# Vigilans/GomokuAI

Measured on AMD Instinct MI355X. Metric: board-evals/s, higher is better.
Workload: dtype int32

## Files before the change

gomokuai_amd/csrc/eval_kernel.hip:

```cpp
#include <algorithm>
#include <cstdlib>
#include <vector>

#include "capi_common.h"

namespace {

constexpr int kBoardsPerBlock = 16;
constexpr int kGroupBoards = 16;
constexpr int kThreads = 64 * kBoardsPerBlock;
constexpr int kCells = 225;
constexpr int kQueueCap = 448;
constexpr int kMaxBlocksPerCu = 1;

constexpr int kScoreWords = 4 * kCells;
constexpr int kCntWords = 3 * kCells + 1;
constexpr int kZeroWords = kScoreWords + kCntWords;
constexpr int kLineWords = 96;
constexpr int kColBase = 20, kDiagBase = 36, kAntiBase = 65;
#ifndef GMK_K1_TOTALS_COPIES
#define GMK_K1_TOTALS_COPIES 8
#endif
constexpr int kTotalsCopies = GMK_K1_TOTALS_COPIES;
constexpr int kMiscWords = 48;
constexpr int kBoardWords = kZeroWords + kLineWords + kQueueCap + kMiscWords;
static_assert(kZeroWords % 4 == 0 && kBoardWords % 4 == 0, "16-byte alignment of the per-board blocks");
constexpr int kStaticTableWords = 128 + kLineWords + 512 + 1560 + 4;

__constant__ uint32_t c_lane_jobs[64 * 2];
__constant__ uint32_t c_line_init[kLineWords];
__constant__ uint4 c_lane_consts[64];
constexpr int kScanSteps = 19;

__device__ __forceinline__ int dir_stride(int dir) { return (0x0E100F01u >> (8 * dir)) & 0xFFu; }

__device__ __forceinline__ uint64_t line_symbols(uint32_t line_word, int len) {
    return 2ull | (static_cast<uint64_t>(line_word) << 2) | (0xAull << (2 * len + 2));
}

__device__ __forceinline__ const __attribute__((address_space(3))) uint32_t* lds_word(uint32_t byte_address) {
    return reinterpret_cast<const __attribute__((address_space(3))) uint32_t*>(static_cast<uintptr_t>(byte_address));
}

__device__ __forceinline__ __attribute__((address_space(3))) uint32_t* lds_word_rw(uint32_t byte_address) {
    return reinterpret_cast<__attribute__((address_space(3))) uint32_t*>(static_cast<uintptr_t>(byte_address));
}

__device__ __forceinline__ uint32_t dfa_address(uint32_t table_word, uint32_t four) {
    uint32_t addr;
    asm("v_bfi_b32 %0, %1, %2, %3" : "=v"(addr) : "s"(0x3FF3u), "v"(table_word), "v"(four));
// ... 57 lines not shown

__device__ __forceinline__ void add_counter_cells(uint32_t w0, int back, int q, int stride, uint32_t* opp) {
    const int n_dep = (w0 >> 8) & 7, endcell = q + back * stride;
#pragma unroll
    for (int d = 0; d < 4; ++d) {
        const uint32_t f = (w0 >> (11 + 4 * d)) & 15u;
        if (d < n_dep && static_cast<int>(f & 7u) != back) atomicAdd(&opp[4 * (endcell - static_cast<int>(f & 7u) * stride)], 600u);
    }
}

[[maybe_unused]] constexpr int kDensTiles = 7;
__host__ __device__ constexpr int dens_kt_lo(int m) { return (((32 * m) / 15 - 3) < 0 ? 0 : (32 * m) / 15 - 3) / 2; }
__host__ __device__ constexpr int dens_kt_hi(int m) { return (((32 * m + 31) / 15 + 3) > 14 ? 14 : (32 * m + 31) / 15 + 3) / 2; }
constexpr int kWtabDy = 13, kWtabEntryWords = 4, kWtabKindWords = kWtabDy * 15 * kWtabEntryWords, kWtabWords = 2 * kWtabKindWords;
__host__ __device__ constexpr int block_weight(int dy, int dx) {
    constexpr int w[4][7] = {{1, 3, 4, 0, 4, 3, 1}, {0, 3, 5, 4, 5, 3, 0}, {0, 4, 3, 3, 3, 4, 0}, {2, 0, 0, 1, 0, 0, 2}};
    return w[dy < 0 ? -dy : dy][dx + 3];
}

typedef int v4i __attribute__((ext_vector_type(4)));
typedef int v16i __attribute__((ext_vector_type(16)));

template <bool kFull, int KIND, int M>
__device__ __forceinline__ void density_tile_pass(const uint32_t (&own_rows)[8], int n_live, int lane,
                                                  const v4i* __restrict__ s_wtab, const uint4* __restrict__ s_occ, int32_t* __restrict__ group_out,
                                                  unsigned long long& board_base , const uint2* __restrict__ s_lut, int plane_stride) {
    constexpr int lo = dens_kt_lo(M), hi = dens_kt_hi(M), nk = hi - lo + 1;
    const int n = lane & 31, h = lane >> 5;
    const uint4 occ_lo = s_occ[4 * M + 2 * h], occ_hi = s_occ[4 * M + 2 * h + 1];
    const uint32_t occ[8] = {occ_lo.x, occ_lo.y, occ_lo.z, occ_lo.w, occ_hi.x, occ_hi.y, occ_hi.z, occ_hi.w};
    const int cell = 32 * M + n, yo = (cell * 0x8889) >> 19, xo = cell - 15 * yo;
    const v4i* w = s_wtab + KIND * (kWtabKindWords / kWtabEntryWords) + (2 * lo + h - yo + 6) * 15 + xo;
    v16i acc = {0, 0, 0, 0, 0, 0, 0, 0, 0, 0, 0, 0, 0, 0, 0, 0};
#pragma unroll
    for (int k = 0; k < nk; ++k) {
        const uint32_t r = (own_rows[lo + k] >> (16 * h)) & 0x7FFFu;
        const uint2 b0 = s_lut[r & 255u], b1 = s_lut[r >> 8];
        const v4i stones = {static_cast<int>(b0.x), static_cast<int>(b0.y), static_cast<int>(b1.x), static_cast<int>(b1.y)};
        acc = __builtin_amdgcn_mfma_i32_32x32x32_i8(stones, w[30 * k], acc, 0, 0, 0);
    }
    const uint32_t at = static_cast<uint32_t>(KIND * plane_stride + 32 * M + n + h * (2 * 4 * plane_stride));
    if (kFull) {
        const uint32_t at_white = 4u * at, at_black = 4u * (at + 2u * static_cast<uint32_t>(plane_stride));
#pragma unroll
        for (int i = 0; i < 16; i += 2) {
            const int neg = __builtin_amdgcn_sbfe(static_cast<int>(occ[i / 2]), n, 1);
            store_saddr(at_black, acc[i] ^ neg, board_base);
            store_saddr(at_white, acc[i + 1] ^ neg, board_base);
            board_base += static_cast<long long>(i == 14 ? -13 : i % 4 ? 3 : 1) * (4 * 4 * plane_stride);
            asm volatile("" : "+s"(board_base));
        }
    } else {
        int32_t* out = group_out + at;
#pragma unroll
        for (int i = 0; i < 16; i += 2) {
            const int b = 4 * (i / 4) + (i % 4) / 2;
            const int neg = __builtin_amdgcn_sbfe(static_cast<int>(occ[i / 2]), n, 1);
            asm volatile("" : "+s"(n_live));
            if (b + 2 * h < n_live && plane_stride > 0) {
                out[b * 4 * plane_stride + 1 * 2 * plane_stride] = acc[i] ^ neg;
                out[b * 4 * plane_stride + 0 * 2 * plane_stride] = acc[i + 1] ^ neg;
            }
        }
    }
}

template <bool kFull>
__device__ __forceinline__ void density_planes_out(const uint16_t* __restrict__ planes, int n_boards, int first_board, int lane,
                                                   const v4i* __restrict__ s_wtab, uint32_t* __restrict__ s_occ, int32_t* __restrict__ out_density,
                                                   const uint2* __restrict__ s_lut, int plane_stride) {
    const int n = lane & 31, plane = n & 1, board = first_board + (n >> 1);
    uint32_t own[8], other[8];
    {
        const uint4* p = reinterpret_cast<const uint4*>(planes + static_cast<size_t>(kFull || board < n_boards ? board : first_board) * 32);
        const uint4 a0 = p[plane * 2], a1 = p[plane * 2 + 1], b0 = p[2 - plane * 2], b1 = p[3 - plane * 2];
        own[0] = a0.x; own[1] = a0.y; own[2] = a0.z; own[3] = a0.w; own[4] = a1.x; own[5] = a1.y; own[6] = a1.z; own[7] = a1.w;
        other[0] = b0.x; other[1] = b0.y; other[2] = b0.z; other[3] = b0.w; other[4] = b1.x; other[5] = b1.y; other[6] = b1.z; other[7] = b1.w;
    }
    if ((lane & 33) == 0) {
        const int bg = lane >> 1;
        uint32_t* slot = s_occ + 8 * ((bg >> 1) & 1) + 2 * (bg >> 2) + (bg & 1);
#pragma unroll
        for (int m = 0; m < kDensTiles; ++m) {
            const int y0 = (32 * m) / 15, y1 = (32 * m + 31) / 15;
            uint32_t occ = 0;
#pragma unroll
            for (int y = y0; y <= y1; ++y) {
                const uint32_t both = own[y / 2] | other[y / 2];
                const uint32_t r = ((y & 1) ? both >> 16 : both) & 0x7FFFu;
                const int at = 15 * y - 32 * m;
                occ |= at >= 0 ? r << at : r >> -at;
            }
            slot[16 * m] = occ;
        }
    }
    if ((lane >> 5) == 0 && (kFull || (board < n_boards && plane_stride > 0))) {
        uint32_t c224 = 0, w224 = 0;
#pragma unroll
        for (int dy = -3; dy <= 0; ++dy) {
            const int y = 14 + dy;
            const uint32_t r = (y & 1) ? own[y >> 1] >> 16 : own[y >> 1] & 0xFFFFu;
#pragma unroll
            for (int dx = -3; dx <= 0; ++dx) {
                if (block_weight(dy, dx) == 0) continue;
                const uint32_t bit = (r >> (14 + dx)) & 1u;
                c224 += bit;
                w224 += bit * static_cast<uint32_t>(block_weight(dy, dx));
            }
        }
        const uint32_t neg = 0u - (((own[7] | other[7]) >> 14) & 1u);
        int32_t* out = out_density + static_cast<size_t>(board) * 4 * plane_stride + (1 - plane) * 2 * plane_stride;
        out[224] = static_cast<int32_t>(c224 ^ neg);
        out[plane_stride + 224] = static_cast<int32_t>(w224 ^ neg);
    }
    const int n_live = __builtin_amdgcn_readfirstlane(n_boards - first_board);
    int32_t* group_out = out_density + static_cast<size_t>(first_board) * 4 * plane_stride;
    const uint4* occ_words = reinterpret_cast<const uint4*>(s_occ);
    const unsigned long long group_bits = reinterpret_cast<unsigned long long>(group_out);
    unsigned long long board_base = static_cast<unsigned long long>(static_cast<uint32_t>(__builtin_amdgcn_readfirstlane(static_cast<int>(group_bits >> 32)))) << 32
                                    | static_cast<uint32_t>(__builtin_amdgcn_readfirstlane(static_cast<int>(group_bits)));
    asm volatile("" : "+s"(board_base));
#define GMK_PASS(K, M) density_tile_pass<kFull, K, M>(own, n_live, lane, s_wtab, occ_words, group_out, board_base, s_lut, plane_stride); __builtin_amdgcn_sched_barrier(0);
    GMK_PASS(0, 0) GMK_PASS(1, 0) GMK_PASS(0, 1) GMK_PASS(1, 1) GMK_PASS(0, 2) GMK_PASS(1, 2) GMK_PASS(0, 3) GMK_PASS(1, 3)
    GMK_PASS(0, 4) GMK_PASS(1, 4) GMK_PASS(0, 5) GMK_PASS(1, 5) GMK_PASS(0, 6) GMK_PASS(1, 6)
#undef GMK_PASS
}

__global__ __launch_bounds__(kThreads)
void eval_positions_kernel(const uint16_t* __restrict__ planes, int n_boards, int n_groups,
                           int32_t* __restrict__ out_scores, int32_t* __restrict__ out_density,
                           uint32_t* __restrict__ out_totals, int32_t* __restrict__ out_status,
                           const uint32_t* __restrict__ g_trans, const uint32_t* __restrict__ g_records,
                           int trans_words, int record_words, const uint32_t* __restrict__ g_wtab,
                           int phase_mask_arg, unsigned long long* __restrict__ prof) {
#ifdef GMK_PROFILE
    const int phase_mask = phase_mask_arg;
    unsigned long long t_acc[12] = {0, 0, 0, 0, 0, 0, 0, 0, 0, 0, 0, 0}, t_prev = __builtin_amdgcn_s_memtime();
#define GMK_STAMP(k) do { if (prof) { const unsigned long long t_now_ = __builtin_amdgcn_s_memtime(); t_acc[k] += t_now_ - t_prev; t_prev = t_now_; } } while (0)
#else
    constexpr int phase_mask = 0x7F;
    (void)phase_mask_arg; (void)prof;
#define GMK_STAMP(k) do { } while (0)
#endif
    extern __shared__ __attribute__((aligned(16))) uint32_t lds[];
    const uint4* s_rec = reinterpret_cast<const uint4*>(lds + trans_words);
    uint32_t* s_jobs = lds + trans_words + record_words;

    for (int i = threadIdx.x; i < trans_words; i += kThreads) lds[i] = g_trans[i];
    for (int i = threadIdx.x; i < record_words; i += kThreads) lds[trans_words + i] = g_records[i];
    if (threadIdx.x < 128) s_jobs[threadIdx.x] = c_lane_jobs[threadIdx.x];
    uint32_t* s_pads = s_jobs + 128;
    if (threadIdx.x < kLineWords) s_pads[threadIdx.x] = ~c_line_init[threadIdx.x] & 0xAAAAAAAAu;
    uint2* s_lut = reinterpret_cast<uint2*>(s_jobs + 128 + kLineWords);
    if (threadIdx.x < 256) s_lut[threadIdx.x] = make_uint2(((threadIdx.x & 15u) * 0x204081u) & 0x01010101u, ((threadIdx.x >> 4) * 0x204081u) & 0x01010101u);
    uint32_t* s_wtab_words = s_jobs + 128 + kLineWords + 512;
    for (int i = threadIdx.x; i < kWtabWords; i += kThreads) s_wtab_words[i] = g_wtab[i];
    const v4i* s_wtab = reinterpret_cast<const v4i*>(s_wtab_words);
    uint32_t* s_handout = s_wtab_words + kWtabWords;
    if (threadIdx.x < 4) s_handout[threadIdx.x] = threadIdx.x == 0 ? 2u * kBoardsPerBlock : 0u;

    const int wave = __builtin_amdgcn_readfirstlane(threadIdx.x >> 6), lane0 = threadIdx.x & 63;
    uint32_t* s_scores = lds + trans_words + record_words + kStaticTableWords + wave * kBoardWords;
    uint32_t* s_cnt = s_scores + kScoreWords;
    uint32_t* s_lines = s_scores + kZeroWords;
    uint32_t* s_queue = s_lines + kLineWords;
    uint32_t* s_misc = s_queue + kQueueCap;
#ifndef GMK_K1_TOTALS_HOT
    uint32_t* const my_totals = s_queue + kQueueCap - 8 * kTotalsCopies + (lane0 & (kTotalsCopies - 1)) * 8;
#else
    uint32_t* const my_totals = s_misc + 4;
#endif

    GMK_STAMP(0);

    const bool planes_out = out_density != nullptr && (phase_mask & 64) && !(phase_mask & 1024);
    int lane = lane0;
    const uint32_t job_a = c_lane_jobs[lane * 2], job_b = c_lane_jobs[lane * 2 + 1];
    const uint32_t line_init_lo = c_line_init[lane], line_init_hi = c_line_init[min(64 + lane, kLineWords - 1)];
    const uint4 lane_consts = c_lane_consts[lane];
    const uint32_t cell_row4 = lane_consts.x, cell_col = lane_consts.y, norm_a = lane_consts.z, norm_b = lane_consts.w;
    uint32_t* s_rows = s_misc + 16;
    const uint16_t* row_ptr = planes + (lane & 15);
    uint32_t next_black = 0, next_white = 0, cur_black = 0, cur_white = 0;
    auto fetch_row = [&](int b) {
        const uint16_t* p = row_ptr + static_cast<size_t>(min(b, n_boards - 1)) * 32;
        next_black = p[0];
        next_white = p[16];
    };
    auto take_row = [&](int b) -> uint32_t { return lane < 16 && b < n_boards ? cur_black | (cur_white << 16) : 0u; };

    const int wg_g0 = static_cast<int>(static_cast<long long>(n_groups) * blockIdx.x / gridDim.x);
    const int wg_groups = static_cast<int>(static_cast<long long>(n_groups) * (blockIdx.x + 1) / gridDim.x) - wg_g0;
    const int wg_first = wg_g0 * kGroupBoards, wg_boards = min(wg_groups * kGroupBoards, n_boards - wg_first);
    auto hand_out = [&](int which) -> int {
        uint32_t v = 0;
        if (lane0 == 0) v = atomicAdd(&s_handout[which], 1u);
        return __builtin_amdgcn_readfirstlane(static_cast<int>(v));
    };
    int idx = wave, boards_done = 0;
    if (idx < wg_boards) fetch_row(wg_first + idx);
    asm volatile("" : "+v"(next_black), "+v"(next_white));
#pragma unroll 1
    for (;;) {
        const bool live = idx < wg_boards;
        const int board = wg_first + idx;
        cur_black = next_black; cur_white = next_white;
        int idx_next = idx;
        if (live) { idx_next = boards_done == 0 ? kBoardsPerBlock + wave : hand_out(0); fetch_row(wg_first + min(idx_next, wg_boards - 1)); }
        GMK_STAMP(11);

        if (live) {
            {
                uint4* z = reinterpret_cast<uint4*>(s_cnt) + lane;
    #pragma unroll
                for (int i = 0; i < kCntWords / 4; i += 64)
                    if (i + 64 <= kCntWords / 4 || lane < kCntWords / 4 - i) z[i] = make_uint4(0u, 0u, 0u, 0u);
            }
            s_lines[lane] = line_init_lo;
            if (lane < kLineWords - 64) s_lines[64 + lane] = line_init_hi;
            if (lane < kMiscWords) s_misc[lane] = 0;
#ifndef GMK_K1_TOTALS_HOT
            if (lane < 8 * kTotalsCopies) s_queue[kQueueCap - 8 * kTotalsCopies + lane] = 0;
#endif
            const uint32_t my_row = take_row(board);
            wave_phase_fence();
            {
                uint32_t cnt = static_cast<uint32_t>(__popc(my_row & 0x7FFFu)) | (static_cast<uint32_t>(__popc(my_row >> 16)) << 16);
                cnt += static_cast<uint32_t>(__builtin_amdgcn_update_dpp(0, static_cast<int>(cnt), 0x118, 0xF, 0xF, false));
                cnt += static_cast<uint32_t>(__builtin_amdgcn_update_dpp(0, static_cast<int>(cnt), 0x114, 0xF, 0xF, false));
                cnt += static_cast<uint32_t>(__builtin_amdgcn_update_dpp(0, static_cast<int>(cnt), 0x112, 0xF, 0xF, false));
                cnt += static_cast<uint32_t>(__builtin_amdgcn_update_dpp(0, static_cast<int>(cnt), 0x111, 0xF, 0xF, false));
// ... 230 lines not shown
                        for (int i = 0; i < 8; ++i)
                            if (start + i <= k) tw = *lds_word(dfa_address(tw, __builtin_amdgcn_ubfe(cur, 2 * i, 4)));
                        if ((gmk::dev_trans_kinds(tw) >> tslot) & 1u) {
                            const uint4 rec = s_rec[gmk::dev_trans_record(tw)];
                            const int want = 5 - tslot;
                            hit_back = counter_match(rec.x, k, want);
                            hit_w0 = rec.x;
                            if (hit_back < 0) { hit_back = counter_match(rec.z, k, want); hit_w0 = rec.z; }
                        }
                    }
                    const unsigned long long hits = __ballot(hit_back >= 0);
                    const uint32_t mine = static_cast<uint32_t>(hits >> (7 * grp)) & 0x7Fu;
                    if (hit_back >= 0 && (mine & ((1u << kk) - 1u)) == 0u) add_counter_cells(hit_w0, hit_back, q, stride, s_scores + (c ? 2 : 1));
                }
            }
            wave_phase_fence();
            GMK_STAMP(6);

        }

        asm volatile("" : "+v"(next_black), "+v"(next_white));
        GMK_STAMP(7);

        if (planes_out && (!live || (boards_done & 15) == wave)) {
            for (;;) {
                const int burst = hand_out(1);
                if (burst >= wg_groups) break;
                int lane_p = lane0, first_p = (wg_g0 + burst) * kGroupBoards;
                asm volatile("" : "+v"(lane_p), "+s"(first_p));
                const int plane_stride = (phase_mask & 512) ? 0 : (phase_mask & 256) ? 256 : kCells;
                if (first_p + kGroupBoards <= n_boards && plane_stride > 0) density_planes_out<true>(planes, n_boards, first_p, lane_p, s_wtab, s_queue, out_density, s_lut, plane_stride);
                else density_planes_out<false>(planes, n_boards, first_p, lane_p, s_wtab, s_queue, out_density, s_lut, plane_stride);
                GMK_STAMP(8);
                if (live) break;
            }
        }
        if (!live) break;
        if (live && (phase_mask & 32)) {
            int lane_b = lane;
            asm volatile("" : "+v"(lane_b));
            if (out_scores) {
                int32_t* dst = out_scores + static_cast<size_t>(board) * kScoreWords + lane_b;
                const int4* src = reinterpret_cast<const int4*>(s_scores);
                const int4 v0 = src[lane_b], v1 = src[lane_b + 64], v2 = src[lane_b + 128], v3 = src[min(lane_b + 192, kCells - 1)];
#ifdef GMK_K1_PLAIN_SCORES
#define GMK_STORE(p, v) (*(p) = (v))
#else
#define GMK_STORE(p, v) __builtin_nontemporal_store(v, p)
#endif
                const bool tail = lane_b + 192 < kCells;
                GMK_STORE(dst, v0.x); GMK_STORE(dst + 64, v1.x); GMK_STORE(dst + 128, v2.x); if (tail) GMK_STORE(dst + 192, v3.x);
                GMK_STORE(dst + kCells, v0.y); GMK_STORE(dst + kCells + 64, v1.y); GMK_STORE(dst + kCells + 128, v2.y); if (tail) GMK_STORE(dst + kCells + 192, v3.y);
                GMK_STORE(dst + 2 * kCells, v0.z); GMK_STORE(dst + 2 * kCells + 64, v1.z); GMK_STORE(dst + 2 * kCells + 128, v2.z); if (tail) GMK_STORE(dst + 2 * kCells + 192, v3.z);
                GMK_STORE(dst + 3 * kCells, v0.w); GMK_STORE(dst + 3 * kCells + 64, v1.w); GMK_STORE(dst + 3 * kCells + 128, v2.w); if (tail) GMK_STORE(dst + 3 * kCells + 192, v3.w);
#undef GMK_STORE
            }
            if (out_totals && lane_b < 11) out_totals[static_cast<size_t>(board) * 11 + lane_b] = s_misc[4 + lane_b];
            if (out_status && lane_b == 0) {
                const uint32_t wbits = s_misc[1], stones = s_misc[0];
// ... 73 lines not shown
            for (int xo = 0; xo < 15; ++xo)
                for (int j = 0; j < 15; ++j) {
                    if (std::abs(j - xo) > 3) continue;
                    const int w = block_weight(dy, j - xo);
                    t[((static_cast<size_t>(kind) * kWtabDy + dy + 6) * 15 + xo) * 16 + j] = static_cast<int8_t>(kind == 0 ? (w != 0) : w);
                }
    for (int cell = 0; cell < 224; ++cell)
        for (int kt = dens_kt_lo(cell / 32); kt <= dens_kt_hi(cell / 32); ++kt)
            for (int h = 0; h < 2; ++h) {
                const int dy = 2 * kt + h - cell / 15;
                if (dy < -6 || dy > 6) { gmk::set_error("density weight table: dy %d of cell %d out of range", dy, cell); return GMK_ERR_STATE; }
            }
    for (int cell = 0; cell < 224; ++cell)
        for (int dy = -3; dy <= 3; ++dy) {
            const int y = cell / 15 + dy, m = cell / 32;
            if (y < 0 || y > 14) continue;
            if (y / 2 < dens_kt_lo(m) || y / 2 > dens_kt_hi(m)) { gmk::set_error("density weight table: row %d of cell %d is not covered", y, cell); return GMK_ERR_STATE; }
        }
    GMK_HIP_CHECK(hipMalloc(d_out, t.size()));
    GMK_HIP_CHECK(hipMemcpy(*d_out, t.data(), t.size(), hipMemcpyHostToDevice));
    return GMK_OK;
}

struct Launch { int grid, n_groups; size_t lds; };

Launch plan_launch(int n, const gmk::DeviceState& st) {
    Launch l;
    l.n_groups = (n + kGroupBoards - 1) / kGroupBoards;
    l.grid = std::max(1, std::min(l.n_groups, st.cu_count * kMaxBlocksPerCu));
    l.lds = static_cast<size_t>(kBoardsPerBlock * kBoardWords + st.n_states * 4 + st.n_records * 4 + kStaticTableWords) * 4;
    return l;
}

bool g_jobs_uploaded = false;
uint32_t* g_wtab = nullptr;
}

extern "C" int gmk_eval_batch(const uint16_t* d_planes, int n, int32_t* d_scores, int32_t* d_density,
                              uint32_t* d_totals, int32_t* d_status, void* stream) {
    gmk::DeviceState& st = gmk::device_state();
    if (!st.ready) { gmk::set_error("gmk_init has not succeeded (no CPU fallback)"); return GMK_ERR_STATE; }
    if (n < 0 || (n > 0 && !d_planes)) { gmk::set_error("gmk_eval_batch: bad arguments"); return GMK_ERR_ARG; }
    if (n == 0) return GMK_OK;
    if (!g_jobs_uploaded) {
        int rc = upload_lane_jobs();
        if (rc != GMK_OK) return rc;
        rc = upload_density_weights(&g_wtab);
        if (rc != GMK_OK) return rc;
        GMK_HIP_CHECK(hipFuncSetAttribute(reinterpret_cast<const void*>(eval_positions_kernel), hipFuncAttributeMaxDynamicSharedMemorySize, 160 * 1024));
        g_jobs_uploaded = true;
    }
    const Launch l = plan_launch(n, st);
    if (l.lds > 160u * 1024u) { gmk::set_error("gmk_eval_batch: tables do not fit in LDS (%zu bytes)", l.lds); return GMK_ERR_CAPACITY; }
    static const int phase_mask = gmk::profile_env("GMK_EVAL_PHASE_MASK") ? std::atoi(gmk::profile_env("GMK_EVAL_PHASE_MASK")) : 0x7F;
    unsigned long long* d_prof = nullptr;
    static const bool stamps = gmk::profile_env("GMK_EVAL_PROFILE") != nullptr;
    if (stamps) {
        GMK_HIP_CHECK(hipMalloc(&d_prof, 16 * sizeof(unsigned long long)));
        GMK_HIP_CHECK(hipMemset(d_prof, 0, 16 * sizeof(unsigned long long)));
    }
    hipLaunchKernelGGL(eval_positions_kernel, dim3(l.grid), dim3(kThreads), l.lds, static_cast<hipStream_t>(stream),
                       d_planes, n, l.n_groups, d_scores, d_density, d_totals, d_status,
                       st.d_trans, st.d_records, st.n_states * 4, st.n_records * 4, g_wtab, phase_mask, d_prof);
    GMK_HIP_CHECK(hipGetLastError());
    if (stamps) {
        unsigned long long h[16];
        GMK_HIP_CHECK(hipDeviceSynchronize());
        GMK_HIP_CHECK(hipMemcpy(h, d_prof, sizeof h, hipMemcpyDeviceToHost));
        (void)hipFree(d_prof);
        const char* names[12] = {"staging", "phase0", "scan", "deposits", "phase3", "phase3b", "rescans", "wait-planes", "phaseD", "phase5", "-", "loop-head"};
        const double boards = static_cast<double>(n), waves = static_cast<double>(h[15] ? h[15] : 1);
        double total = 0;
        for (int k = 0; k < 12; ++k) total += static_cast<double>(h[k]);
        std::fprintf(stderr, "[GMK_EVAL_PROFILE] s_memtime cycles per board (wavefront time; %.0f wavefronts, %.0f cycles each):", waves, total / waves);
        for (int k = 0; k < 12; ++k) if (k != 10) std::fprintf(stderr, " %s %.0f", names[k], static_cast<double>(h[k]) / boards);
        std::fprintf(stderr, "\n");
    }
    return GMK_OK;
}

extern "C" int gmk_eval_launch_info(int n, int* grid, int* block, int* lds_bytes) {
    gmk::DeviceState& st = gmk::device_state();
    if (!st.ready) { gmk::set_error("gmk_init has not succeeded"); return GMK_ERR_STATE; }
    const Launch l = plan_launch(std::max(n, 1), st);
    if (grid) *grid = l.grid;
    if (block) *block = kThreads;
    if (lds_bytes) *lds_bytes = static_cast<int>(l.lds);
    return GMK_OK;
}

extern "C" int gmk_eval_batch_host(const uint16_t* h_planes, int n, int32_t* h_scores, int32_t* h_density,
                                   uint32_t* h_totals, int32_t* h_status) {
    gmk::DeviceState& st = gmk::device_state();
    if (!st.ready) { gmk::set_error("gmk_init has not succeeded (no CPU fallback)"); return GMK_ERR_STATE; }
    if (n < 0 || (n > 0 && !h_planes)) { gmk::set_error("gmk_eval_batch_host: bad arguments"); return GMK_ERR_ARG; }
    if (n == 0) return GMK_OK;
    uint16_t* d_planes = nullptr;
    int32_t *d_scores = nullptr, *d_density = nullptr, *d_status = nullptr;
    uint32_t* d_totals = nullptr;
    const size_t nb = static_cast<size_t>(n);
    int rc = GMK_OK;
    auto cleanup = [&]() { (void)hipFree(d_planes); (void)hipFree(d_scores); (void)hipFree(d_density); (void)hipFree(d_totals); (void)hipFree(d_status); };
#define GMK_TRY(expr) do { if ((expr) != hipSuccess) { gmk::set_error("%s failed", #expr); cleanup(); return GMK_ERR_HIP; } } while (0)
    GMK_TRY(hipMalloc(&d_planes, nb * 64));
    GMK_TRY(hipMalloc(&d_scores, nb * 3600));
    GMK_TRY(hipMalloc(&d_density, nb * 3600));
    GMK_TRY(hipMalloc(&d_totals, nb * 44));
    GMK_TRY(hipMalloc(&d_status, nb * 4));
    GMK_TRY(hipMemcpy(d_planes, h_planes, nb * 64, hipMemcpyHostToDevice));
    rc = gmk_eval_batch(d_planes, n, d_scores, d_density, d_totals, d_status, nullptr);
// ... 11 lines not shown
```

gomokuai_amd/lib.py:

```python
import ctypes as C
import os

import numpy as np

_HERE = os.path.dirname(os.path.abspath(__file__))
_SO = os.path.join(_HERE, "libgomoku_hip.so")
if os.environ.get("GMK_HIP_LIB") == "prof":
    _SO = os.path.join(_HERE, "libgomoku_hip_prof.so")
elif os.environ.get("GMK_HIP_LIB", "").endswith(".so"):
    _SO = os.environ["GMK_HIP_LIB"]

N = 225


class GmkError(RuntimeError):
    pass


class TableInfo(C.Structure):
    _fields_ = [("n_patterns", C.c_int32), ("n_states", C.c_int32), ("dat_size", C.c_int32),
                ("max_emissions", C.c_int32), ("trans_words", C.c_int32), ("emit_words", C.c_int32),
                ("invariants", C.c_int32 * 5)]


_lib = None

OPT_NOISE_SAMPLER, OPT_LOCKSTEP = 1, 2
NOISE_SAMPLERS = {"std": 0, "counter": 1}

EXPORTS = [
    "gmk_init", "gmk_shutdown", "gmk_pool_release", "gmk_pool_poison", "gmk_last_error", "gmk_device_info",
    "gmk_tables_info", "gmk_tables_pattern", "gmk_tables_copy", "gmk_tables_copy_dat", "gmk_tables_scan",
    "gmk_synth_boards", "gmk_moves_to_planes",
    "gmk_eval_batch", "gmk_eval_batch_host", "gmk_eval_launch_info",
    "gmk_mcts_create", "gmk_mcts_destroy", "gmk_mcts_set_roots", "gmk_mcts_set_game_ids", "gmk_mcts_run", "gmk_mcts_root_stats",
    "gmk_mcts_alg_bytes", "gmk_mcts_launch_info", "gmk_visits_to_pi", "gmk_mcts_advance", "gmk_mcts_step", "gmk_mcts_step_host", "gmk_mcts_add_root_noise", "gmk_mcts_set_option", "gmk_mcts_reserve", "gmk_selfplay_run", "gmk_samples_from_records",
    "gmk_records_scan", "gmk_records_packed_bytes", "gmk_records_pack", "gmk_records_unpack", "gmk_samples_from_packed",
    "gmk_evalstate_create", "gmk_evalstate_destroy", "gmk_evalstate_reset", "gmk_evalstate_update", "gmk_evalstate_update_host", "gmk_evalstate_read",
    "gmk_az_create", "gmk_az_destroy", "gmk_az_set_roots", "gmk_az_select", "gmk_az_expand", "gmk_az_select_host", "gmk_az_expand_host", "gmk_az_read_node_host", "gmk_az_read_children_host", "gmk_az_set_leaf_host", "gmk_az_rollout_host", "gmk_az_expand_stages_host", "gmk_az_write_stats_host", "gmk_az_step", "gmk_az_advance", "gmk_az_set_slots", "gmk_az_live_games", "gmk_az_set_game_ids", "gmk_az_add_root_noise", "gmk_az_set_option", "gmk_az_root_stats",
    "gmk_trad_create", "gmk_trad_destroy", "gmk_trad_reset_evaluators", "gmk_trad_set_game_ids", "gmk_trad_set_positions", "gmk_trad_run", "gmk_trad_step", "gmk_trad_add_root_noise", "gmk_trad_set_option", "gmk_trad_reserve", "gmk_trad_root_stats", "gmk_trad_read_evaluators", "gmk_trad_run_poolrave", "gmk_trad_run_rave", "gmk_trad_root_amaf", "gmk_trad_selfplay_run", "gmk_pvnet_create", "gmk_pvnet_destroy", "gmk_pvnet_forward", "gmk_pvnet_set_dense", "gmk_pvnet_evaluate",
]


def _torch_first():
    try:
        import torch
    except ImportError:
        return
    if torch.cuda.is_available():
        torch.cuda.init()


def load():
    global _lib
    if _lib is not None:
        return _lib
    _torch_first()
    if not os.path.exists(_SO):
        raise GmkError("libgomoku_hip.so is missing: run `python -m gomokuai_amd.build` "
                       "(there is no CPU fallback for the compute path)")
    L = C.CDLL(_SO)
    vp = C.c_void_p
    L.gmk_last_error.restype = C.c_char_p
    L.gmk_init.argtypes = [C.c_int]
    L.gmk_device_info.argtypes = [C.POINTER(C.c_int), C.POINTER(C.c_size_t), C.c_char_p, C.c_int]
    L.gmk_tables_info.argtypes = [C.POINTER(TableInfo)]
    L.gmk_tables_pattern.argtypes = [C.c_int, C.c_char_p, C.POINTER(C.c_int), C.POINTER(C.c_int), C.POINTER(C.c_int)]
    L.gmk_tables_copy.argtypes = [vp, vp, vp]
    L.gmk_tables_copy_dat.argtypes = [vp, vp, vp]
    L.gmk_tables_scan.argtypes = [vp, C.c_int, vp, vp, C.c_int]
    L.gmk_synth_boards.argtypes = [C.c_uint64, C.c_uint32, C.c_int, C.c_int, vp, C.c_int, vp, vp]
    L.gmk_moves_to_planes.argtypes = [vp, C.c_int, vp, C.c_int, vp]
    L.gmk_eval_batch.argtypes = [vp, C.c_int, vp, vp, vp, vp, vp]
    L.gmk_eval_batch_host.argtypes = [vp, C.c_int, vp, vp, vp, vp]
    L.gmk_eval_launch_info.argtypes = [C.c_int, C.POINTER(C.c_int), C.POINTER(C.c_int), C.POINTER(C.c_int)]
    L.gmk_mcts_create.argtypes = [C.c_int, C.c_int, C.c_double, C.c_int, C.c_uint64, C.POINTER(vp)]
    L.gmk_mcts_destroy.argtypes = [vp]
    L.gmk_mcts_set_roots.argtypes = [vp, vp, vp, C.c_uint32]
    L.gmk_mcts_set_game_ids.argtypes = [vp, vp]
    L.gmk_trad_set_game_ids.argtypes = [vp, vp]
    L.gmk_az_set_game_ids.argtypes = [vp, vp]
    L.gmk_mcts_run.argtypes = [vp, C.c_int, vp]
    L.gmk_mcts_root_stats.argtypes = [vp, vp, vp, vp, vp, vp]
    L.gmk_mcts_alg_bytes.argtypes = [vp, C.POINTER(C.c_uint64)]
    L.gmk_mcts_launch_info.argtypes = [vp, C.POINTER(C.c_int), C.POINTER(C.c_int), C.POINTER(C.c_int)]
    L.gmk_visits_to_pi.argtypes = [vp, C.c_int, vp]
    L.gmk_mcts_advance.argtypes = [vp, vp, vp, vp, vp, vp, C.c_int, vp]
    L.gmk_mcts_step.argtypes = [vp, vp, vp, vp, vp, vp, vp, C.c_int, vp]
    L.gmk_mcts_step_host.argtypes = [vp, vp, C.c_int]
    L.gmk_selfplay_run.argtypes = [vp, C.c_int, C.c_uint32, C.c_int, C.c_int, C.c_float, C.c_float, vp, C.c_int, vp, vp, vp, vp, vp, C.POINTER(C.c_int32), vp]
    L.gmk_mcts_add_root_noise.argtypes = [vp, C.c_float, C.c_float, vp]
    L.gmk_mcts_set_option.argtypes = [vp, C.c_int, C.c_int]
    L.gmk_mcts_reserve.argtypes = [vp, C.c_int]
    L.gmk_trad_reserve.argtypes = [vp, C.c_int]
    L.gmk_evalstate_create.argtypes = [C.c_int, C.POINTER(vp)]
    L.gmk_evalstate_destroy.argtypes = [vp]
    L.gmk_evalstate_reset.argtypes = [vp]
    L.gmk_evalstate_update.argtypes = [vp, vp, C.c_int, vp]
# ... 131 lines not shown
def eval_batch_host(planes):
    init()
    planes = np.ascontiguousarray(planes, dtype=np.uint16)
    n = planes.shape[0]
    scores = np.zeros((n, 4, N), dtype=np.int32)
    density = np.zeros((n, 2, 2, N), dtype=np.int32)
    totals = np.zeros((n, 11), dtype=np.uint32)
    status = np.zeros(n, dtype=np.int32)
    _check(load().gmk_eval_batch_host(planes.ctypes.data, n, scores.ctypes.data, density.ctypes.data,
                                      totals.ctypes.data, status.ctypes.data))
    return scores, density, totals, status


def eval_batch(d_planes, n, d_scores=None, d_density=None, d_totals=None, d_status=None, stream=None):
    _check(load().gmk_eval_batch(d_planes, n, d_scores, d_density, d_totals, d_status, stream))


def eval_launch_info(n):
    g, b, l = C.c_int(), C.c_int(), C.c_int()
    _check(load().gmk_eval_launch_info(n, C.byref(g), C.byref(b), C.byref(l)))
    return {"grid": g.value, "block": b.value, "lds_bytes": l.value}


class BatchedMCTS:

    def __init__(self, n_games, playouts_capacity=800, c_puct=5.0, c_rollouts=5, seed=DEFAULT_SEED, node_capacity=None):
        init()
        self.n = n_games
        self.cap = node_capacity if node_capacity is not None else playouts_capacity * 225 + 1
        h = C.c_void_p()
        _check(load().gmk_mcts_create(n_games, self.cap, c_puct, c_rollouts, seed, C.byref(h)))
        self.h = h

    def close(self):
        if getattr(self, "h", None) and load is not None:
            load().gmk_mcts_destroy(self.h)
            self.h = None

    __del__ = close

    def set_roots(self, planes, last_moves, first_game_id=0):
        planes = np.ascontiguousarray(planes, dtype=np.uint16)
        last = np.ascontiguousarray(last_moves, dtype=np.int16)
        assert planes.shape == (self.n, 2, 16) and last.shape == (self.n,)
        _check(load().gmk_mcts_set_roots(self.h, planes.ctypes.data, last.ctypes.data, first_game_id))

# ... 388 lines not shown
```

include/gomoku_hip.h:

```cpp
#ifndef GOMOKU_HIP_H_
#define GOMOKU_HIP_H_
#include <stddef.h>
#include <stdint.h>

#ifdef __cplusplus
extern "C" {
#endif

typedef enum {
    GMK_OK = 0,
    GMK_ERR_NO_DEVICE = -1,
    GMK_ERR_HIP = -2,
    GMK_ERR_ARG = -3,
    GMK_ERR_STATE = -4,
    GMK_ERR_CAPACITY = -5
} gmk_status;

enum { GMK_BOARD_CELLS = 225, GMK_PLANE_WORDS = 16, GMK_TOTALS = 11 };

int gmk_init(int device);
int gmk_shutdown(void);
int gmk_pool_release(void);
int gmk_pool_poison(int on);
const char *gmk_last_error(void);
// ... 4 lines not shown
    int32_t n_states;
    int32_t dat_size;
    int32_t max_emissions;
    int32_t trans_words;
    int32_t emit_words;
    int32_t invariants[5];
} gmk_table_info;
int gmk_tables_info(gmk_table_info *info);
int gmk_tables_pattern(int i, char str[8], int *favour, int *type, int *score);
int gmk_tables_copy(uint32_t *trans, uint16_t *emit_lists, uint32_t *pattern_info);
int gmk_tables_copy_dat(int32_t *base, int32_t *check, int32_t *fail);
int gmk_tables_scan(const uint8_t *codes, int n, int32_t *patterns, int32_t *offsets, int cap);

int gmk_synth_boards(uint64_t seed, uint32_t first_board, int n, int kind,
                     uint8_t *h_moves, int stride, int32_t *h_lens, uint16_t *h_planes);
int gmk_moves_to_planes(const uint8_t *h_moves, int stride, const int32_t *h_lens, int n, uint16_t *h_planes);

int gmk_eval_batch(const uint16_t *d_planes, int n,
                   int32_t *d_scores, int32_t *d_density, uint32_t *d_totals, int32_t *d_status,
                   void *stream);
int gmk_eval_batch_host(const uint16_t *h_planes, int n,
                        int32_t *h_scores, int32_t *h_density, uint32_t *h_totals, int32_t *h_status);
int gmk_eval_launch_info(int n, int *grid, int *block, int *lds_bytes);

typedef struct gmk_evalstate gmk_evalstate;
int gmk_evalstate_create(int n_games, gmk_evalstate **out);
int gmk_evalstate_destroy(gmk_evalstate *e);
int gmk_evalstate_reset(gmk_evalstate *e);
int gmk_evalstate_update(gmk_evalstate *e, const int16_t *d_moves, int moves_per_game, void *stream);
int gmk_evalstate_update_host(gmk_evalstate *e, const int16_t *h_moves, int moves_per_game);
int gmk_evalstate_read(gmk_evalstate *e, int32_t *h_scores, int32_t *h_density, uint32_t *h_pattern_dist, uint32_t *h_compound_dist,
                       int32_t *h_meta, uint8_t *h_record);

typedef struct gmk_mcts gmk_mcts;
int gmk_mcts_create(int n_games, int node_capacity, double c_puct, int c_rollouts, uint64_t seed, gmk_mcts **out);
int gmk_mcts_destroy(gmk_mcts *m);
int gmk_mcts_set_roots(gmk_mcts *m, const uint16_t *h_planes, const int16_t *h_last_move, uint32_t first_game_id);
int gmk_mcts_set_game_ids(gmk_mcts *m, const uint32_t *h_ids);
int gmk_mcts_run(gmk_mcts *m, int playouts, void *stream);
int gmk_mcts_advance(gmk_mcts *m, uint8_t *d_moves, uint16_t *d_visits, int32_t *d_lens, int8_t *d_winner,
                     int32_t *d_unfinished, int reuse_subtree, void *stream);
int gmk_selfplay_run(gmk_mcts *m, int n_total, uint32_t first_game_id, int playouts, int reuse_subtree, float noise_alpha, float noise_epsilon,
                     const uint8_t *h_open_moves, int open_stride, const int32_t *h_open_lens,
                     uint8_t *d_moves, uint16_t *d_visits, int32_t *d_lens, int8_t *d_winner, int32_t *h_steps, void *stream);
int gmk_mcts_step(gmk_mcts* m, const int16_t* d_forced_moves, uint8_t* d_moves, uint16_t* d_visits, int32_t* d_lens,
                  int8_t* d_winner, int32_t* d_unfinished, int reuse_subtree, void* stream);
// ... 93 lines not shown
```

Measured before the change: 548.4 million.

## Split density planes into separate kernel on side stream overlapping eval kernel

Moves the MFMA density-plane computation out of the main eval kernel into its own 4-wave kernel, launched on a non-blocking side stream with fork and join events so it can run alongside the pattern-scan kernel. The eval kernel sheds its LUT and weight-table LDS, and the launch check now makes sure both kernels' LDS fit on a CU together. Stone expansion uses mul24 bit tricks instead of an LDS lookup and is computed once per group rather than per tile pass. The risk is that the two kernels compete for CU resources, and the event synchronisation adds per-call overhead.

```diff
diff --git a/gomokuai_amd/csrc/eval_kernel.hip b/gomokuai_amd/csrc/eval_kernel.hip
--- a/gomokuai_amd/csrc/eval_kernel.hip
+++ b/gomokuai_amd/csrc/eval_kernel.hip
@@ -25,7 +25,7 @@
 constexpr int kMiscWords = 48;
 constexpr int kBoardWords = kZeroWords + kLineWords + kQueueCap + kMiscWords;
 static_assert(kZeroWords % 4 == 0 && kBoardWords % 4 == 0, "16-byte alignment of the per-board blocks");
-constexpr int kStaticTableWords = 128 + kLineWords + 512 + 1560 + 4;
+constexpr int kStaticTableWords = 128 + kLineWords + 4;
 
 __constant__ uint32_t c_lane_jobs[64 * 2];
 __constant__ uint32_t c_line_init[kLineWords];
@@ -129,9 +129,9 @@
 typedef int v16i __attribute__((ext_vector_type(16)));
 
 template <bool kFull, int KIND, int M>
-__device__ __forceinline__ void density_tile_pass(const uint32_t (&own_rows)[8], int n_live, int lane,
+__device__ __forceinline__ void density_tile_pass(const v4i (&stones)[8], int n_live, int lane,
                                                   const v4i* __restrict__ s_wtab, const uint4* __restrict__ s_occ, int32_t* __restrict__ group_out,
-                                                  unsigned long long& board_base , const uint2* __restrict__ s_lut, int plane_stride) {
+                                                  unsigned long long& board_base , int plane_stride) {
     constexpr int lo = dens_kt_lo(M), hi = dens_kt_hi(M), nk = hi - lo + 1;
     const int n = lane & 31, h = lane >> 5;
     const uint4 occ_lo = s_occ[4 * M + 2 * h], occ_hi = s_occ[4 * M + 2 * h + 1];
@@ -140,12 +140,7 @@
     const v4i* w = s_wtab + KIND * (kWtabKindWords / kWtabEntryWords) + (2 * lo + h - yo + 6) * 15 + xo;
     v16i acc = {0, 0, 0, 0, 0, 0, 0, 0, 0, 0, 0, 0, 0, 0, 0, 0};
 #pragma unroll
-    for (int k = 0; k < nk; ++k) {
-        const uint32_t r = (own_rows[lo + k] >> (16 * h)) & 0x7FFFu;
-        const uint2 b0 = s_lut[r & 255u], b1 = s_lut[r >> 8];
-        const v4i stones = {static_cast<int>(b0.x), static_cast<int>(b0.y), static_cast<int>(b1.x), static_cast<int>(b1.y)};
-        acc = __builtin_amdgcn_mfma_i32_32x32x32_i8(stones, w[30 * k], acc, 0, 0, 0);
-    }
+    for (int k = 0; k < nk; ++k) acc = __builtin_amdgcn_mfma_i32_32x32x32_i8(stones[lo + k], w[30 * k], acc, 0, 0, 0);
     const uint32_t at = static_cast<uint32_t>(KIND * plane_stride + 32 * M + n + h * (2 * 4 * plane_stride));
     if (kFull) {
         const uint32_t at_white = 4u * at, at_black = 4u * (at + 2u * static_cast<uint32_t>(plane_stride));
@@ -175,7 +170,7 @@
 template <bool kFull>
 __device__ __forceinline__ void density_planes_out(const uint16_t* __restrict__ planes, int n_boards, int first_board, int lane,
                                                    const v4i* __restrict__ s_wtab, uint32_t* __restrict__ s_occ, int32_t* __restrict__ out_density,
-                                                   const uint2* __restrict__ s_lut, int plane_stride) {
+                                                   int plane_stride) {
     const int n = lane & 31, plane = n & 1, board = first_board + (n >> 1);
     uint32_t own[8], other[8];
     {
@@ -220,6 +215,16 @@
         out[224] = static_cast<int32_t>(c224 ^ neg);
         out[plane_stride + 224] = static_cast<int32_t>(w224 ^ neg);
     }
+    v4i stones[8];
+    {
+        const int h = lane >> 5;
+#pragma unroll
+        for (int kt = 0; kt < 8; ++kt) {
+            const uint32_t r = (own[kt] >> (16 * h)) & 0x7FFFu;
+            stones[kt] = v4i{static_cast<int>(mul24(r & 15u, 0x204081u) & 0x01010101u), static_cast<int>(mul24((r >> 4) & 15u, 0x204081u) & 0x01010101u),
+                             static_cast<int>(mul24((r >> 8) & 15u, 0x204081u) & 0x01010101u), static_cast<int>(mul24(r >> 12, 0x204081u) & 0x01010101u)};
+        }
+    }
     const int n_live = __builtin_amdgcn_readfirstlane(n_boards - first_board);
     int32_t* group_out = out_density + static_cast<size_t>(first_board) * 4 * plane_stride;
     const uint4* occ_words = reinterpret_cast<const uint4*>(s_occ);
@@ -227,18 +232,57 @@
     unsigned long long board_base = static_cast<unsigned long long>(static_cast<uint32_t>(__builtin_amdgcn_readfirstlane(static_cast<int>(group_bits >> 32)))) << 32
                                     | static_cast<uint32_t>(__builtin_amdgcn_readfirstlane(static_cast<int>(group_bits)));
     asm volatile("" : "+s"(board_base));
-#define GMK_PASS(K, M) density_tile_pass<kFull, K, M>(own, n_live, lane, s_wtab, occ_words, group_out, board_base, s_lut, plane_stride); __builtin_amdgcn_sched_barrier(0);
+#define GMK_PASS(K, M) density_tile_pass<kFull, K, M>(stones, n_live, lane, s_wtab, occ_words, group_out, board_base, plane_stride); __builtin_amdgcn_sched_barrier(0);
     GMK_PASS(0, 0) GMK_PASS(1, 0) GMK_PASS(0, 1) GMK_PASS(1, 1) GMK_PASS(0, 2) GMK_PASS(1, 2) GMK_PASS(0, 3) GMK_PASS(1, 3)
     GMK_PASS(0, 4) GMK_PASS(1, 4) GMK_PASS(0, 5) GMK_PASS(1, 5) GMK_PASS(0, 6) GMK_PASS(1, 6)
 #undef GMK_PASS
 }
 
+constexpr int kDensWaves = 4, kDensThreads = 64 * kDensWaves;
+constexpr int kDensOccWords = kDensTiles * 16;
+constexpr int kDensLdsBytes = (kWtabWords + kDensWaves * kDensOccWords + 4) * 4;
+
+__global__ __launch_bounds__(kDensThreads) __attribute__((amdgpu_waves_per_eu(4)))
+void density_planes_kernel(const uint16_t* __restrict__ planes, int n_boards, int n_groups, int32_t* __restrict__ out_density,
+                           const uint32_t* __restrict__ g_wtab, int plane_stride_arg) {
+#ifdef GMK_PROFILE
+    const int plane_stride = plane_stride_arg;
+#else
+    constexpr int plane_stride = kCells;
+    (void)plane_stride_arg;
+#endif
+    __shared__ __attribute__((aligned(16))) uint32_t s_wtab_words[kWtabWords];
+    __shared__ __attribute__((aligned(16))) uint32_t s_occ_words[kDensWaves * kDensOccWords];
+    __shared__ uint32_t s_handout[4];
+    static_assert(sizeof(s_wtab_words) + sizeof(s_occ_words) + sizeof(s_handout) == kDensLdsBytes, "gmk_eval_split_info reports this size");
+    for (int i = threadIdx.x; i < kWtabWords; i += kDensThreads) s_wtab_words[i] = g_wtab[i];
+    if (threadIdx.x == 0) s_handout[0] = 0u;
+    __syncthreads();
+    const int wave = __builtin_amdgcn_readfirstlane(threadIdx.x >> 6), lane = threadIdx.x & 63;
+    const v4i* s_wtab = reinterpret_cast<const v4i*>(s_wtab_words);
+    uint32_t* s_occ = s_occ_words + wave * kDensOccWords;
+    const int wg_g0 = static_cast<int>(static_cast<long long>(n_groups) * blockIdx.x / gridDim.x);
+    const int wg_groups = static_cast<int>(static_cast<long long>(n_groups) * (blockIdx.x + 1) / gridDim.x) - wg_g0;
+#pragma unroll 1
+    for (;;) {
+        uint32_t v = 0;
+        if (lane == 0) v = atomicAdd(&s_handout[0], 1u);
+        const int burst = __builtin_amdgcn_readfirstlane(static_cast<int>(v));
+        if (burst >= wg_groups) break;
+        int lane_p = lane, first = (wg_g0 + burst) * kGroupBoards;
+        asm volatile("" : "+v"(lane_p), "+s"(first));
+        if (first + kGroupBoards <= n_boards && plane_stride > 0) density_planes_out<true>(planes, n_boards, first, lane_p, s_wtab, s_occ, out_density, plane_stride);
+        else density_planes_out<false>(planes, n_boards, first, lane_p, s_wtab, s_occ, out_density, plane_stride);
+        wave_phase_fence();
+    }
+}
+
 __global__ __launch_bounds__(kThreads)
 void eval_positions_kernel(const uint16_t* __restrict__ planes, int n_boards, int n_groups,
-                           int32_t* __restrict__ out_scores, int32_t* __restrict__ out_density,
+                           int32_t* __restrict__ out_scores,
                            uint32_t* __restrict__ out_totals, int32_t* __restrict__ out_status,
                            const uint32_t* __restrict__ g_trans, const uint32_t* __restrict__ g_records,
-                           int trans_words, int record_words, const uint32_t* __restrict__ g_wtab,
+                           int trans_words, int record_words,
                            int phase_mask_arg, unsigned long long* __restrict__ prof) {
 #ifdef GMK_PROFILE
     const int phase_mask = phase_mask_arg;
@@ -258,12 +302,7 @@
     if (threadIdx.x < 128) s_jobs[threadIdx.x] = c_lane_jobs[threadIdx.x];
     uint32_t* s_pads = s_jobs + 128;
     if (threadIdx.x < kLineWords) s_pads[threadIdx.x] = ~c_line_init[threadIdx.x] & 0xAAAAAAAAu;
-    uint2* s_lut = reinterpret_cast<uint2*>(s_jobs + 128 + kLineWords);
-    if (threadIdx.x < 256) s_lut[threadIdx.x] = make_uint2(((threadIdx.x & 15u) * 0x204081u) & 0x01010101u, ((threadIdx.x >> 4) * 0x204081u) & 0x01010101u);
-    uint32_t* s_wtab_words = s_jobs + 128 + kLineWords + 512;
-    for (int i = threadIdx.x; i < kWtabWords; i += kThreads) s_wtab_words[i] = g_wtab[i];
-    const v4i* s_wtab = reinterpret_cast<const v4i*>(s_wtab_words);
-    uint32_t* s_handout = s_wtab_words + kWtabWords;
+    uint32_t* s_handout = s_jobs + 128 + kLineWords;
     if (threadIdx.x < 4) s_handout[threadIdx.x] = threadIdx.x == 0 ? 2u * kBoardsPerBlock : 0u;
 
     const int wave = __builtin_amdgcn_readfirstlane(threadIdx.x >> 6), lane0 = threadIdx.x & 63;
@@ -280,7 +319,6 @@
 
     GMK_STAMP(0);
 
-    const bool planes_out = out_density != nullptr && (phase_mask & 64) && !(phase_mask & 1024);
     int lane = lane0;
     const uint32_t job_a = c_lane_jobs[lane * 2], job_b = c_lane_jobs[lane * 2 + 1];
     const uint32_t line_init_lo = c_line_init[lane], line_init_hi = c_line_init[min(64 + lane, kLineWords - 1)];
@@ -299,9 +337,9 @@
     const int wg_g0 = static_cast<int>(static_cast<long long>(n_groups) * blockIdx.x / gridDim.x);
     const int wg_groups = static_cast<int>(static_cast<long long>(n_groups) * (blockIdx.x + 1) / gridDim.x) - wg_g0;
     const int wg_first = wg_g0 * kGroupBoards, wg_boards = min(wg_groups * kGroupBoards, n_boards - wg_first);
-    auto hand_out = [&](int which) -> int {
+    auto hand_out = [&]() -> int {
         uint32_t v = 0;
-        if (lane0 == 0) v = atomicAdd(&s_handout[which], 1u);
+        if (lane0 == 0) v = atomicAdd(&s_handout[0], 1u);
         return __builtin_amdgcn_readfirstlane(static_cast<int>(v));
     };
     int idx = wave, boards_done = 0;
@@ -313,7 +351,7 @@
         const int board = wg_first + idx;
         cur_black = next_black; cur_white = next_white;
         int idx_next = idx;
-        if (live) { idx_next = boards_done == 0 ? kBoardsPerBlock + wave : hand_out(0); fetch_row(wg_first + min(idx_next, wg_boards - 1)); }
+        if (live) { idx_next = boards_done == 0 ? kBoardsPerBlock + wave : hand_out(); fetch_row(wg_first + min(idx_next, wg_boards - 1)); }
         GMK_STAMP(11);
 
         if (live) {
@@ -590,19 +628,6 @@
         asm volatile("" : "+v"(next_black), "+v"(next_white));
         GMK_STAMP(7);
 
-        if (planes_out && (!live || (boards_done & 15) == wave)) {
-            for (;;) {
-                const int burst = hand_out(1);
-                if (burst >= wg_groups) break;
-                int lane_p = lane0, first_p = (wg_g0 + burst) * kGroupBoards;
-                asm volatile("" : "+v"(lane_p), "+s"(first_p));
-                const int plane_stride = (phase_mask & 512) ? 0 : (phase_mask & 256) ? 256 : kCells;
-                if (first_p + kGroupBoards <= n_boards && plane_stride > 0) density_planes_out<true>(planes, n_boards, first_p, lane_p, s_wtab, s_queue, out_density, s_lut, plane_stride);
-                else density_planes_out<false>(planes, n_boards, first_p, lane_p, s_wtab, s_queue, out_density, s_lut, plane_stride);
-                GMK_STAMP(8);
-                if (live) break;
-            }
-        }
         if (!live) break;
         if (live && (phase_mask & 32)) {
             int lane_b = lane;
@@ -722,18 +747,25 @@
     return GMK_OK;
 }
 
-struct Launch { int grid, n_groups; size_t lds; };
+struct Launch { int grid, n_groups; size_t lds; int dens_grid; };
 
 Launch plan_launch(int n, const gmk::DeviceState& st) {
     Launch l;
     l.n_groups = (n + kGroupBoards - 1) / kGroupBoards;
     l.grid = std::max(1, std::min(l.n_groups, st.cu_count * kMaxBlocksPerCu));
     l.lds = static_cast<size_t>(kBoardsPerBlock * kBoardWords + st.n_states * 4 + st.n_records * 4 + kStaticTableWords) * 4;
+    l.dens_grid = std::max(1, std::min(l.n_groups, st.cu_count));
     return l;
 }
+
+constexpr size_t kLdsPerCu = 160u * 1024u, kLdsGranule = 1280u;
+constexpr size_t lds_alloc(size_t bytes) { return (bytes + kLdsGranule - 1) / kLdsGranule * kLdsGranule; }
 
 bool g_jobs_uploaded = false;
 uint32_t* g_wtab = nullptr;
+int g_fork_device = -1;
+hipStream_t g_side_stream = nullptr;
+hipEvent_t g_fork_event = nullptr, g_join_event = nullptr;
 }
 
 extern "C" int gmk_eval_batch(const uint16_t* d_planes, int n, int32_t* d_scores, int32_t* d_density,
@@ -748,10 +780,18 @@
         rc = upload_density_weights(&g_wtab);
         if (rc != GMK_OK) return rc;
         GMK_HIP_CHECK(hipFuncSetAttribute(reinterpret_cast<const void*>(eval_positions_kernel), hipFuncAttributeMaxDynamicSharedMemorySize, 160 * 1024));
+        GMK_HIP_CHECK(hipStreamCreateWithFlags(&g_side_stream, hipStreamNonBlocking));
+        GMK_HIP_CHECK(hipEventCreateWithFlags(&g_fork_event, hipEventDisableTiming));
+        GMK_HIP_CHECK(hipEventCreateWithFlags(&g_join_event, hipEventDisableTiming));
+        g_fork_device = st.device;
         g_jobs_uploaded = true;
     }
+    if (g_fork_device != st.device) { gmk::set_error("gmk_eval_batch: tables were uploaded on device %d, now on %d", g_fork_device, st.device); return GMK_ERR_STATE; }
     const Launch l = plan_launch(n, st);
-    if (l.lds > 160u * 1024u) { gmk::set_error("gmk_eval_batch: tables do not fit in LDS (%zu bytes)", l.lds); return GMK_ERR_CAPACITY; }
+    if (lds_alloc(l.lds) + lds_alloc(kDensLdsBytes) > kLdsPerCu) {
+        gmk::set_error("gmk_eval_batch: tables do not fit in LDS (%zu + %d bytes)", l.lds, kDensLdsBytes);
+        return GMK_ERR_CAPACITY;
+    }
     static const int phase_mask = gmk::profile_env("GMK_EVAL_PHASE_MASK") ? std::atoi(gmk::profile_env("GMK_EVAL_PHASE_MASK")) : 0x7F;
     unsigned long long* d_prof = nullptr;
     static const bool stamps = gmk::profile_env("GMK_EVAL_PROFILE") != nullptr;
@@ -759,21 +799,34 @@
         GMK_HIP_CHECK(hipMalloc(&d_prof, 16 * sizeof(unsigned long long)));
         GMK_HIP_CHECK(hipMemset(d_prof, 0, 16 * sizeof(unsigned long long)));
     }
-    hipLaunchKernelGGL(eval_positions_kernel, dim3(l.grid), dim3(kThreads), l.lds, static_cast<hipStream_t>(stream),
-                       d_planes, n, l.n_groups, d_scores, d_density, d_totals, d_status,
-                       st.d_trans, st.d_records, st.n_states * 4, st.n_records * 4, g_wtab, phase_mask, d_prof);
+    hipStream_t s = static_cast<hipStream_t>(stream);
+    const bool fork = d_density != nullptr && (phase_mask & 64) && !(phase_mask & 1024);
+    if (fork) {
+        GMK_HIP_CHECK(hipEventRecord(g_fork_event, s));
+        GMK_HIP_CHECK(hipStreamWaitEvent(g_side_stream, g_fork_event, 0));
+        hipLaunchKernelGGL(density_planes_kernel, dim3(l.dens_grid), dim3(kDensThreads), 0, g_side_stream,
+                           d_planes, n, l.n_groups, d_density, g_wtab, (phase_mask & 512) ? 0 : (phase_mask & 256) ? 256 : kCells);
+        GMK_HIP_CHECK(hipGetLastError());
+    }
+    hipLaunchKernelGGL(eval_positions_kernel, dim3(l.grid), dim3(kThreads), l.lds, s,
+                       d_planes, n, l.n_groups, d_scores, d_totals, d_status,
+                       st.d_trans, st.d_records, st.n_states * 4, st.n_records * 4, phase_mask, d_prof);
     GMK_HIP_CHECK(hipGetLastError());
+    if (fork) {
+        GMK_HIP_CHECK(hipEventRecord(g_join_event, g_side_stream));
+        GMK_HIP_CHECK(hipStreamWaitEvent(s, g_join_event, 0));
+    }
     if (stamps) {
         unsigned long long h[16];
         GMK_HIP_CHECK(hipDeviceSynchronize());
         GMK_HIP_CHECK(hipMemcpy(h, d_prof, sizeof h, hipMemcpyDeviceToHost));
         (void)hipFree(d_prof);
-        const char* names[12] = {"staging", "phase0", "scan", "deposits", "phase3", "phase3b", "rescans", "wait-planes", "phaseD", "phase5", "-", "loop-head"};
+        const char* names[12] = {"staging", "phase0", "scan", "deposits", "phase3", "phase3b", "rescans", "wait-planes", "-", "phase5", "-", "loop-head"};
         const double boards = static_cast<double>(n), waves = static_cast<double>(h[15] ? h[15] : 1);
         double total = 0;
         for (int k = 0; k < 12; ++k) total += static_cast<double>(h[k]);
         std::fprintf(stderr, "[GMK_EVAL_PROFILE] s_memtime cycles per board (wavefront time; %.0f wavefronts, %.0f cycles each):", waves, total / waves);
-        for (int k = 0; k < 12; ++k) if (k != 10) std::fprintf(stderr, " %s %.0f", names[k], static_cast<double>(h[k]) / boards);
+        for (int k = 0; k < 12; ++k) if (k != 8 && k != 10) std::fprintf(stderr, " %s %.0f", names[k], static_cast<double>(h[k]) / boards);
         std::fprintf(stderr, "\n");
     }
     return GMK_OK;
@@ -786,6 +839,18 @@
     if (grid) *grid = l.grid;
     if (block) *block = kThreads;
     if (lds_bytes) *lds_bytes = static_cast<int>(l.lds);
+    return GMK_OK;
+}
+
+extern "C" int gmk_eval_split_info(int n, int* eval_lds_bytes, int* density_grid, int* density_block, int* density_lds_bytes, int* lds_granule_bytes) {
+    gmk::DeviceState& st = gmk::device_state();
+    if (!st.ready) { gmk::set_error("gmk_init has not succeeded"); return GMK_ERR_STATE; }
+    const Launch l = plan_launch(std::max(n, 1), st);
+    if (eval_lds_bytes) *eval_lds_bytes = static_cast<int>(l.lds);
+    if (density_grid) *density_grid = l.dens_grid;
+    if (density_block) *density_block = kDensThreads;
+    if (density_lds_bytes) *density_lds_bytes = kDensLdsBytes;
+    if (lds_granule_bytes) *lds_granule_bytes = static_cast<int>(kLdsGranule);
     return GMK_OK;
 }
 
diff --git a/gomokuai_amd/lib.py b/gomokuai_amd/lib.py
--- a/gomokuai_amd/lib.py
+++ b/gomokuai_amd/lib.py
@@ -32,7 +32,7 @@
     "gmk_init", "gmk_shutdown", "gmk_pool_release", "gmk_pool_poison", "gmk_last_error", "gmk_device_info",
     "gmk_tables_info", "gmk_tables_pattern", "gmk_tables_copy", "gmk_tables_copy_dat", "gmk_tables_scan",
     "gmk_synth_boards", "gmk_moves_to_planes",
-    "gmk_eval_batch", "gmk_eval_batch_host", "gmk_eval_launch_info",
+    "gmk_eval_batch", "gmk_eval_batch_host", "gmk_eval_launch_info", "gmk_eval_split_info",
     "gmk_mcts_create", "gmk_mcts_destroy", "gmk_mcts_set_roots", "gmk_mcts_set_game_ids", "gmk_mcts_run", "gmk_mcts_root_stats",
     "gmk_mcts_alg_bytes", "gmk_mcts_launch_info", "gmk_visits_to_pi", "gmk_mcts_advance", "gmk_mcts_step", "gmk_mcts_step_host", "gmk_mcts_add_root_noise", "gmk_mcts_set_option", "gmk_mcts_reserve", "gmk_selfplay_run", "gmk_samples_from_records",
     "gmk_records_scan", "gmk_records_packed_bytes", "gmk_records_pack", "gmk_records_unpack", "gmk_samples_from_packed",
@@ -74,6 +74,7 @@
     L.gmk_eval_batch.argtypes = [vp, C.c_int, vp, vp, vp, vp, vp]
     L.gmk_eval_batch_host.argtypes = [vp, C.c_int, vp, vp, vp, vp]
     L.gmk_eval_launch_info.argtypes = [C.c_int, C.POINTER(C.c_int), C.POINTER(C.c_int), C.POINTER(C.c_int)]
+    L.gmk_eval_split_info.argtypes = [C.c_int] + [C.POINTER(C.c_int)] * 5
     L.gmk_mcts_create.argtypes = [C.c_int, C.c_int, C.c_double, C.c_int, C.c_uint64, C.POINTER(vp)]
     L.gmk_mcts_destroy.argtypes = [vp]
     L.gmk_mcts_set_roots.argtypes = [vp, vp, vp, C.c_uint32]
@@ -251,6 +252,12 @@
     return {"grid": g.value, "block": b.value, "lds_bytes": l.value}
 
 
+def eval_split_info(n):
+    v = [C.c_int() for _ in range(5)]
+    _check(load().gmk_eval_split_info(n, *[C.byref(x) for x in v]))
+    return dict(zip(("eval_lds_bytes", "density_grid", "density_block", "density_lds_bytes", "lds_granule_bytes"), (x.value for x in v)))
+
+
 class BatchedMCTS:
 
     def __init__(self, n_games, playouts_capacity=800, c_puct=5.0, c_rollouts=5, seed=DEFAULT_SEED, node_capacity=None):
diff --git a/include/gomoku_hip.h b/include/gomoku_hip.h
--- a/include/gomoku_hip.h
+++ b/include/gomoku_hip.h
@@ -50,6 +50,7 @@
 int gmk_eval_batch_host(const uint16_t *h_planes, int n,
                         int32_t *h_scores, int32_t *h_density, uint32_t *h_totals, int32_t *h_status);
 int gmk_eval_launch_info(int n, int *grid, int *block, int *lds_bytes);
+int gmk_eval_split_info(int n, int *eval_lds_bytes, int *density_grid, int *density_block, int *density_lds_bytes, int *lds_granule_bytes);
 
 typedef struct gmk_evalstate gmk_evalstate;
 int gmk_evalstate_create(int n_games, gmk_evalstate **out);
```

Result: slower. 466.5 million (-14.9%).
